# DIAGNijmegen/spgnn

Measured on NVIDIA B200. Metric: spgnn3_train_graphs_per_s, higher is better.
Workload: dtype f32

## Files before the change

### include/spgnn_b200.h

```cpp
#ifndef SPGNN_B200_H
#define SPGNN_B200_H

#include <stdint.h>

#ifdef __cplusplus
extern "C" {
#endif

#define SPGNN_OK            0
#define SPGNN_E_INVALID    -1
#define SPGNN_E_CUDA       -2
#define SPGNN_E_UNSUPPORTED -3
#define SPGNN_E_WORKSPACE  -4

#define SPGNN_ACT_NONE 0
#define SPGNN_ACT_ELU  1
#define SPGNN_ACT_TANH 2
#define SPGNN_ACT_RELU 3
#define SPGNN_ACT_LEAKY 4

const char* spgnn_last_error(void);
int  spgnn_abi_version(void);
int64_t spgnn_launch_count(void);
int  spgnn_device_info(int* sm_count, int* cc_major, int* cc_minor);
// ... 36 lines not shown
                       float p, uint64_t seed, int64_t concat_chunks, int64_t chunk_off,
                       uint16_t* out_hi, int64_t ldo, int64_t plane_stride, int64_t M, void* stream);
int64_t spgnn_planes_linear_fwd_ws(int64_t N, int64_t K1, int64_t K2);
int spgnn_planes_linear_fwd(const uint16_t* A1, int64_t lda1, int64_t ps1, int64_t K1,
                            const uint16_t* A2, int64_t lda2, int64_t ps2, int64_t K2,
                            const float* W, int64_t ldw, const float* bias, int act, float slope,
                            float* C, int64_t ldc, int64_t M, int64_t N, void* ws, int64_t ws_bytes, void* stream);
int64_t spgnn_planes_linear_bwd_input_ws(int64_t N, int64_t K);
int spgnn_planes_linear_bwd_input(const uint16_t* dC, int64_t lddc, int64_t ps, const float* W, int64_t ldw,
                                  int64_t k_off, float* dA, int64_t ldda, int64_t M, int64_t N, int64_t K,
                                  void* ws, int64_t ws_bytes, void* stream);
int spgnn_planes_linear_bwd_input_masked(const uint16_t* dC, int64_t lddc, int64_t ps, const float* W, int64_t ldw,
                                         int64_t k_off, float* dA, int64_t ldda, int64_t M, int64_t N, int64_t K,
                                         float drop_p, uint64_t seed, int64_t concat_chunks,
                                         void* ws, int64_t ws_bytes, void* stream);
int64_t spgnn_planes_linear_bwd_weight_ws(int64_t M, int64_t N, int64_t K1, int64_t K2);
int spgnn_planes_linear_bwd_weight(const uint16_t* dC, int64_t lddc, int64_t psc,
                                   const uint16_t* X1, int64_t ldx1, int64_t psx1, int64_t K1,
                                   const uint16_t* X2, int64_t ldx2, int64_t psx2, int64_t K2,
                                   float* dW, int64_t lddw, int64_t M, int64_t N,
                                   void* ws, int64_t ws_bytes, void* stream);
int64_t spgnn_act_bwd_planes_ws(int64_t N);
int spgnn_act_bwd_planes(const float* g, int64_t ldg, const float* y, int64_t ldy, int act, float slope,
                         float drop_p, uint64_t drop_seed, uint16_t* out_hi, int64_t ldo, int64_t plane_stride,
                         int64_t M, int64_t N, float* colsum_out, void* ws, void* stream);
int64_t spgnn_planes_linear_bwd_weight_plan(int64_t M, int64_t N, int64_t K1, int64_t K2, int32_t* out, int64_t cap);

int64_t spgnn_colsum_ws(int64_t N);
int spgnn_colsum(const float* X, int64_t ldx, int64_t M, int64_t N, float* out, void* ws, void* stream);

// ... 68 lines not shown
    float* d_eler; int64_t ld_de;
    uint16_t* d_eler_planes; int64_t ld_dep; int64_t ps_dep;
    float* dX; int64_t ld_dx;
} spgnn_gat_wide;
int64_t spgnn_gat_wide_sizeof(void);
int spgnn_gat_aggx_fwd(const spgnn_gat_wide* L, void* stream);
int spgnn_gat_aggx_bwd(const spgnn_gat_wide* L, void* stream);

int64_t spgnn_wide_linear_ws(int64_t H, int64_t F, int64_t kp, int has_res);
int spgnn_wide_linear(const uint16_t* XA, int64_t ldxa, int64_t psxa, int64_t kp, int64_t k_in, int64_t M,
                      int H, int F, int has_res, const float* W, int64_t ldw, const float* bias, int act, int mode,
                      float* out, int64_t ldo, uint16_t* out_planes, int64_t ldp, int64_t psp,
                      const float* g0, int64_t ldg0, const float* g1, int64_t ldg1, const float* g2, int64_t ldg2,
                      uint16_t* dpre, int64_t ldd, int64_t psd, float* dbias,
                      void* ws, int64_t ws_bytes, void* stream);

int spgnn_spmm(const float* x, int64_t ldx, const int32_t* ptr, const int32_t* nbr,
               const float* pre, const float* post, const float* self_eps_ptr,
               const float* bias, int act, float slope,
               float* out, int64_t ldo, int64_t N, int64_t F, void* stream);
int spgnn_degree_norms(const int32_t* ptr, int64_t N, float* norm_sqrt, float* norm_inv, void* stream);

int spgnn_sage_maxpool_fwd(const float* m, int64_t ldm, const int32_t* in_ptr, const int32_t* in_src,
                           float* out, int64_t ldo, int32_t* arg, int64_t N, int64_t F, void* stream);
int spgnn_sage_maxpool_bwd(const float* g, int64_t ldg, const int32_t* arg,
                           const int32_t* out_ptr, const int32_t* out_dst, const int32_t* out_slot,
                           float* dm, int64_t lddm, int64_t N, int64_t F, void* stream);

int spgnn_bias_act(const float* x, int64_t ldx, const float* bias, int act, float slope,
                   float* y, int64_t ldy, int64_t M, int64_t N, void* stream);
// ... 58 lines not shown
```

### spgnn_b200/csrc/gemm_tma.cu

```cuda
#include "common.cuh"
#include "tc_ptx.cuh"

namespace spgnn {
namespace tma {
using namespace ptx;

constexpr int BM = 128;
constexpr int BK = 64;
constexpr int kThreads = 192;
constexpr int kEpiWarps = 4;
constexpr int kMaxStages = 6;
constexpr int kMaxBN = 256;
constexpr int kABytes = BM * 128 * 2;
constexpr int kStgLd = 36;
constexpr int kStgBytes = kEpiWarps * 32 * kStgLd * 4;
constexpr int kSmemLimit = 232448;
constexpr int kNtFixed = 1024  + 256  + kStgBytes;

__device__ __forceinline__ float4 ld_shared4(uint32_t addr) {
    float4 v;
    asm volatile("ld.shared.v4.f32 {%0, %1, %2, %3}, [%4];" : "=f"(v.x), "=f"(v.y), "=f"(v.z), "=f"(v.w) : "r"(addr));
    return v;
}
__device__ __forceinline__ void st_shared4(uint32_t addr, uint32_t a, uint32_t b, uint32_t c, uint32_t d) {
    asm volatile("st.shared.v4.b32 [%0], {%1, %2, %3, %4};" ::"r"(addr), "r"(a), "r"(b), "r"(c), "r"(d) : "memory");
}

struct NtMaps { CUtensorMap a1, a2, b; };
struct NtArgs {
    const float* bias; int act; float slope;
    float* C; int64_t ldc;
    int64_t M; int N;
    int BN, nt_n; int64_t nt_m;
    int kb1, kb2;
    int stages, stage_bytes;
    uint32_t mthr; float mscale; uint64_t mseed; int64_t mnch, moff;
};
__device__ __forceinline__ float4 nt_mask4(const NtArgs& g, float4 x, int64_t row, int col) {
    const uint64_t h = chunk_hash(g.mseed, (uint64_t)row * (uint64_t)g.mnch + (uint64_t)(g.moff + (col >> 2)));
    x.x = ((uint32_t)(h) & 0xFFFFu) >= g.mthr ? x.x * g.mscale : 0.f;
    x.y = ((uint32_t)(h >> 16) & 0xFFFFu) >= g.mthr ? x.y * g.mscale : 0.f;
    x.z = ((uint32_t)(h >> 32) & 0xFFFFu) >= g.mthr ? x.z * g.mscale : 0.f;
    x.w = ((uint32_t)(h >> 48) & 0xFFFFu) >= g.mthr ? x.w * g.mscale : 0.f;
    return x;
}
struct NtShared {
    uint64_t full[kMaxStages];
    uint64_t empty[kMaxStages];
    uint64_t tmem_full[2];
    uint64_t tmem_empty[2];
    uint32_t tmem_base;
// ... 47 lines not shown
                if (g.mthr) x = nt_mask4(g, x, row0 + 4 * itr, col);
                float* qq = q + itr * qstep;
                if (vec_ok && nvalid >= 4) st4(qq, x);
                else {
                    if (nvalid > 0) qq[0] = x.x;
                    if (nvalid > 1) qq[1] = x.y;
                    if (nvalid > 2) qq[2] = x.z;
                    if (nvalid > 3) qq[3] = x.w;
                }
            }
        }
        __syncwarp();
    }
}

template <int CL>
__global__ void __launch_bounds__(kThreads, 1) nt_planes_kernel(const __grid_constant__ NtMaps maps, const NtArgs g) {
    extern __shared__ uint8_t smem_raw[];
    uint8_t* smem = reinterpret_cast<uint8_t*>(((uintptr_t)smem_raw + 1023) & ~(uintptr_t)1023);
    const int stages_bytes = g.stages * g.stage_bytes;
    NtShared* sh = reinterpret_cast<NtShared*>(smem + stages_bytes);
    const int warp = threadIdx.x >> 5, lane = threadIdx.x & 31;
    const uint32_t smem_base = smem_u32(smem);

    if (threadIdx.x == 0) {
        for (int s = 0; s < g.stages; ++s) {
            mbar_init(smem_u32(&sh->full[s]), 1);
            mbar_init(smem_u32(&sh->empty[s]), CL);
        }
        for (int b = 0; b < 2; ++b) {
// ... 12 lines not shown
    __syncthreads();
    if (CL > 1) cluster_sync_all();
    tc_fence_after();
    const uint32_t tmem_base = sh->tmem_base;

    const int rank = CL > 1 ? (int)cluster_ctarank() : 0;
    const int64_t n_tiles = (CL > 1 ? (g.nt_m + CL - 1) / CL : g.nt_m) * g.nt_n;
    const int64_t tile0 = blockIdx.x / CL, tile_step = gridDim.x / CL;
    const int nkb = g.kb1 + g.kb2;

    if (warp < kEpiWarps) {
        int it = 0;
        const uint32_t stg = smem_base + stages_bytes + 256 + warp * (32 * kStgLd * 4);
        const bool vec_ok = (g.ldc % 4 == 0) && ((reinterpret_cast<uintptr_t>(g.C) & 15) == 0);
        const bool plain = (g.act == SPGNN_ACT_NONE) && (g.bias == nullptr);
        for (int64_t tile = tile0; tile < n_tiles; tile += tile_step, ++it) {
            const int buf = it & 1;
            const uint32_t par = (it >> 1) & 1;
            const int64_t m0 = ((tile / g.nt_n) * CL + rank) * BM;
            const int n0 = (int)(tile % g.nt_n) * g.BN;
            const int ncols = min(g.BN, g.N - n0);
            mbar_wait(smem_u32(&sh->tmem_full[buf]), par);
            tc_fence_after();
            const uint32_t taddr = tmem_base + ((uint32_t)(warp * 32) << 16) + (uint32_t)(buf * kMaxBN);
            nt_epilogue_tile(g, stg, taddr, m0, n0, ncols, warp, lane, vec_ok, plain);
            tc_fence_before();
            mbar_arrive(smem_u32(&sh->tmem_empty[buf]));
        }
    } else if (warp == kEpiWarps) {
        {
            int it = 0;
            uint32_t kcount = 0;
            const uint32_t tbase = __shfl_sync(kFull, tmem_base, 0);
            for (int64_t tile = tile0; tile < n_tiles; tile += tile_step, ++it) {
                const int buf = it & 1;
                const uint32_t par = (it >> 1) & 1;
                const int n0 = (int)(tile % g.nt_n) * g.BN;
                const int ncols = min(g.BN, g.N - n0);
                const int n_mma = (ncols + 15) & ~15;
                const uint32_t idesc = make_idesc(n_mma, false);
// ... 187 lines not shown
    if (warp == kEpiWarps) {
        tc_fence_after();
        tmem_dealloc_pair(tmem_base, 512);
    }
}

struct WideMaps { CUtensorMap a, b; };
struct WideArgs {
    int mode, H, F, act;
    const float* bias;
    float* out; int64_t ldo;
    __nv_bfloat16* outp; int64_t ldp, psp;
    const float* g[3]; int64_t ldg[3]; int n_g;
    __nv_bfloat16* dpre; int64_t ldd, psd;
    float* dbias_ws;
    int64_t M; int BN, nt_n; int64_t nt_m;
    int kbp, nparts, kp;
    int stages, stage_bytes;
};
constexpr int kWideEpiWarps = 16;
constexpr int kWideThreads = (kWideEpiWarps + 2) * 32;
constexpr int kWideStgBytes = kWideEpiWarps * 32 * 16 * 4;
constexpr int kWideFixed = 1024  + 256  + kWideStgBytes;

template <int ACT>
__device__ __forceinline__ float wide_act(float x, int act) {
    if (ACT == SPGNN_ACT_ELU) return x > 0.f ? x : exp_fast(x) - 1.f;
    if (ACT == SPGNN_ACT_NONE) return x;
    return act_fwd(x, act, 0.f);
}
template <int ACT>
__device__ __forceinline__ float wide_act_grad(float y, int act) {
    if (ACT == SPGNN_ACT_ELU) return y > 0.f ? 1.f : y + 1.f;
    if (ACT == SPGNN_ACT_NONE) return 1.f;
    return act_grad_from_out(y, act, 0.f);
}
template <int ACT>
__device__ __forceinline__ float wide_act_grad_pre(float x, int act) {
    if (ACT == SPGNN_ACT_ELU) return x > 0.f ? 1.f : exp_fast(x);
    if (ACT == SPGNN_ACT_NONE) return 1.f;
    return act_grad_from_out(act_fwd(x, act, 0.f), act, 0.f);
}
__device__ __forceinline__ void st_planes4(__nv_bfloat16* q, int64_t ps, float4 d) {
    uint32_t h0, l0, h1, l1;
    split2(d.x, d.y, h0, l0);
    split2(d.z, d.w, h1, l1);
    *reinterpret_cast<uint2*>(q) = make_uint2(h0, h1);
    *reinterpret_cast<uint2*>(q + ps) = make_uint2(l0, l1);
}
template <int ACT, int MODE>
__device__ __forceinline__ void wide_epilogue_tile(const WideArgs& g, uint32_t stg, float* dbias_row, uint32_t taddr,
                                                   int64_t m0, int n0, int ncols, int warp, int lane,
                                                   uint32_t full_bar, uint32_t full_par) {
    const int quad = warp & 3, part = warp >> 2;
    const int r0 = lane >> 2, cq = lane & 3;
    const float inv_h = 1.f / (float)g.H;
    const int64_t row0 = m0 + quad * 32 + r0;
    const int nrow = (int)max((int64_t)0, min((int64_t)4, (g.M - row0 + 7) / 8));
    const uint32_t st_w = stg + lane * 64;
    const int sw_w = (lane >> 1) & 3;
    uint32_t st_r[4];
#pragma unroll
    for (int i = 0; i < 4; ++i) {
// ... 35 lines not shown
                for (int i = 0; i < 4; ++i) {
                    run[q][i].x *= inv_h; run[q][i].y *= inv_h; run[q][i].z *= inv_h; run[q][i].w *= inv_h;
                }
        }
        if (cg == 0) {
            mbar_wait(full_bar, full_par);
            tc_fence_after();
        }
#pragma unroll
        for (int q = 0; q < 2; ++q) {
            const int c0 = cg + q * 64 + part * 16;
            if (c0 >= ncols) break;
            const int col = colq + c0;
            __nv_bfloat16* dp = MODE == 1 ? g.dpre + row0 * g.ldd + col : nullptr;
            const int64_t dstep = 8 * g.ldd;
            uint32_t v[16];
            tmem_ld16(taddr + c0, v);
            for (int h = 0; h < g.H; ++h) {
                const float4 bv = g.bias ? ldg4(g.bias + h * g.F + col) : make_float4(0.f, 0.f, 0.f, 0.f);
                tmem_ld_wait();
#pragma unroll
                for (int j = 0; j < 4; ++j)
                    st_shared4(st_w + ((j ^ sw_w) << 4), v[4 * j], v[4 * j + 1], v[4 * j + 2], v[4 * j + 3]);
                __syncwarp();
                if (h + 1 < g.H) tmem_ld16(taddr + (h + 1) * g.BN + c0, v);
                float4 bs = make_float4(0.f, 0.f, 0.f, 0.f);
#pragma unroll
                for (int i = 0; i < 4; ++i) {
                    float4 x = ld_shared4(st_r[i]);
                    if (MODE == 0) {
                        run[q][i].x += wide_act<ACT>(x.x + bv.x, g.act);
                        run[q][i].y += wide_act<ACT>(x.y + bv.y, g.act);
                        run[q][i].z += wide_act<ACT>(x.z + bv.z, g.act);
                        run[q][i].w += wide_act<ACT>(x.w + bv.w, g.act);
                    } else if (i < nrow) {
                        float4 d;
                        d.x = run[q][i].x * wide_act_grad_pre<ACT>(x.x + bv.x, g.act);
                        d.y = run[q][i].y * wide_act_grad_pre<ACT>(x.y + bv.y, g.act);
                        d.z = run[q][i].z * wide_act_grad_pre<ACT>(x.z + bv.z, g.act);
                        d.w = run[q][i].w * wide_act_grad_pre<ACT>(x.w + bv.w, g.act);
                        st_planes4(dp + i * dstep + h * g.F, g.psd, d);
                        bs.x += d.x; bs.y += d.y; bs.z += d.z; bs.w += d.w;
                    }
                }
                if (MODE == 1 && dbias_row) {
#pragma unroll
                    for (int o = 4; o < 32; o <<= 1) {
                        bs.x += __shfl_xor_sync(kFull, bs.x, o); bs.y += __shfl_xor_sync(kFull, bs.y, o);
                        bs.z += __shfl_xor_sync(kFull, bs.z, o); bs.w += __shfl_xor_sync(kFull, bs.w, o);
// ... 782 lines not shown
    const int64_t ldb = k1p + k2p;
    __nv_bfloat16* hi = reinterpret_cast<__nv_bfloat16*>(((uintptr_t)ws + 127) & ~(uintptr_t)127);
    split_weight_kernel<<<split_grid(N * ldb), 256, 0, st>>>(W, ldw, 0, 0, (int)N, (int)ldb, (int)K1, k1p, (int)K2, 0,
                                                             hi, hi + N * ldb, ldb);
    SPGNN_LAUNCH_OK();
    return launch_nt(reinterpret_cast<const __nv_bfloat16*>(A1), lda1, ps1, K1,
                     reinterpret_cast<const __nv_bfloat16*>(A2), lda2, ps2, K2, hi, ldb, bias, act, slope, C, ldc, M, N,
                     st);
}

extern "C" int64_t spgnn_wide_linear_ws(int64_t H, int64_t F, int64_t kp, int has_res) {
    const int64_t b = 2 * H * F * (has_res ? 2 : 1) * kp * (int64_t)sizeof(__nv_bfloat16);
    return b + 256 + (int64_t)sm_count() * H * F * (int64_t)sizeof(float) + 256;
}

extern "C" int spgnn_wide_linear(const uint16_t* XA, int64_t ldxa, int64_t psxa, int64_t kp, int64_t k_in, int64_t M,
                                 int H, int F, int has_res, const float* W, int64_t ldw, const float* bias, int act,
                                 int mode, float* out, int64_t ldo, uint16_t* out_planes, int64_t ldp, int64_t psp,
                                 const float* g0, int64_t ldg0, const float* g1, int64_t ldg1, const float* g2,
                                 int64_t ldg2, uint16_t* dpre, int64_t ldd, int64_t psd, float* dbias, void* ws,
                                 int64_t ws_bytes, void* stream) {
    SPGNN_REQUIRE(XA && W && ws && M > 0 && k_in > 0, "wide_linear: bad argument");
    SPGNN_REQUIRE(H == 1 || H == 2 || H == 4, "wide_linear: H must be 1, 2 or 4 (got %d)", H);
    SPGNN_REQUIRE(F > 0 && F % 32 == 0 && (int64_t)H * F <= 8192, "wide_linear: F (%d) must be a multiple of 32, H*F <= 8192", F);
    SPGNN_REQUIRE(kp % BK == 0 && kp >= k_in && ldxa >= (H + 1) * kp && ldw >= k_in, "wide_linear: kp / ld mismatch");
    SPGNN_REQUIRE(mode == 0 || mode == 1, "wide_linear: mode must be 0 (forward) or 1 (gradient of the pre-activations)");
    SPGNN_REQUIRE(!bias || ((uintptr_t)bias & 15) == 0, "wide_linear: bias must be 16-byte aligned");
    SPGNN_REQUIRE(ws_bytes >= spgnn_wide_linear_ws(H, F, kp, has_res), "wide_linear: workspace too small");
    SPGNN_REQUIRE(M < (1ll << 31), "wide_linear: too many rows");
    WideMaps maps;
    WideArgs a{};
    a.mode = mode; a.H = H; a.F = F; a.act = act; a.bias = bias; a.M = M;
    if (mode == 0) {
        SPGNN_REQUIRE(out || out_planes, "wide_linear: no output");
        SPGNN_REQUIRE(!out || (ldo % 4 == 0 && ldo >= F && ((uintptr_t)out & 15) == 0), "wide_linear: out alignment");
        SPGNN_REQUIRE(!out_planes || (ldp % 4 == 0 && ldp >= F && psp % 4 == 0 && ((uintptr_t)out_planes & 7) == 0),
                      "wide_linear: out planes alignment");
        a.out = out; a.ldo = ldo; a.outp = reinterpret_cast<__nv_bfloat16*>(out_planes); a.ldp = ldp; a.psp = psp;
    } else {
        SPGNN_REQUIRE(g0 && dpre, "wide_linear: mode 1 needs a gradient source and the dpre planes");
        SPGNN_REQUIRE(ldd % 4 == 0 && ldd >= (int64_t)H * F && psd % 4 == 0 && ((uintptr_t)dpre & 7) == 0,
                      "wide_linear: dpre planes alignment");
        const float* gs[3] = {g0, g1, g2};
        const int64_t lds[3] = {ldg0, ldg1, ldg2};
        for (int s = 0; s < 3; ++s) {
            if (!gs[s]) continue;
            SPGNN_REQUIRE(lds[s] % 4 == 0 && lds[s] >= F && ((uintptr_t)gs[s] & 15) == 0,
                          "wide_linear: gradient source %d must be 16-byte aligned with ld %% 4 == 0", s);
            a.g[a.n_g] = gs[s]; a.ldg[a.n_g] = lds[s]; ++a.n_g;
        }
        a.dpre = reinterpret_cast<__nv_bfloat16*>(dpre); a.ldd = ldd; a.psd = psd;
    }
    cudaStream_t st = as_stream(stream);
    static DeviceOnce attr;
// ... 46 lines not shown
        at[0].id = cudaLaunchAttributeClusterDimension;
        at[0].val.clusterDim.x = 2; at[0].val.clusterDim.y = 1; at[0].val.clusterDim.z = 1;
        cfg.gridDim = dim3(grid); cfg.blockDim = dim3(kWideThreads);
        cfg.dynamicSmemBytes = kSmemLimit; cfg.stream = st; cfg.attrs = at; cfg.numAttrs = 1;
        SPGNN_CUDA_OK(cudaLaunchKernelEx(&cfg, wide_pair_kernel, maps, a));
        count_launch();
    } else {
        wide_kernel<<<grid, kWideThreads, kSmemLimit, st>>>(maps, a);
        SPGNN_LAUNCH_OK();
    }
    if (part) {
        wide_dbias_reduce_kernel<<<(unsigned)ceil_div(HF, 128), 128, 0, st>>>(part, grid, HF, dbias);
        SPGNN_LAUNCH_OK();
    }
    return SPGNN_OK;
}

extern "C" int64_t spgnn_planes_linear_bwd_input_ws(int64_t N, int64_t K) {
    return 2 * K * (int64_t)round_up(N, BK) * 2 + 256;
}

extern "C" int spgnn_planes_linear_bwd_input(const uint16_t* dC, int64_t lddc, int64_t ps, const float* W, int64_t ldw,
                                             int64_t k_off, float* dA, int64_t ldda, int64_t M, int64_t N, int64_t K,
                                             void* ws, int64_t ws_bytes, void* stream) {
    return spgnn_planes_linear_bwd_input_masked(dC, lddc, ps, W, ldw, k_off, dA, ldda, M, N, K, 0.f, 0, 0, ws, ws_bytes,
                                                stream);
}

extern "C" int spgnn_planes_linear_bwd_input_masked(const uint16_t* dC, int64_t lddc, int64_t ps, const float* W,
                                                    int64_t ldw, int64_t k_off, float* dA, int64_t ldda, int64_t M,
                                                    int64_t N, int64_t K, float drop_p, uint64_t seed,
                                                    int64_t concat_chunks, void* ws, int64_t ws_bytes, void* stream) {
    SPGNN_REQUIRE(dC && W && dA && ws && M > 0 && N > 0 && K > 0, "planes_linear_bwd_input: bad argument");
    SPGNN_REQUIRE(drop_p >= 0.f && drop_p < 1.f, "planes_linear_bwd_input: dropout p");
    SPGNN_REQUIRE(drop_p == 0.f || k_off % 4 == 0, "planes_linear_bwd_input: a masked output needs k_off %% 4 == 0");
    SPGNN_REQUIRE(ldw >= k_off + K && ldda >= K, "planes_linear_bwd_input: leading dimension too small");
    SPGNN_REQUIRE(ws_bytes >= spgnn_planes_linear_bwd_input_ws(N, K), "planes_linear_bwd_input: workspace too small");
    cudaStream_t st = as_stream(stream);
    const int np = round_up(N, BK);
    __nv_bfloat16* hi = reinterpret_cast<__nv_bfloat16*>(((uintptr_t)ws + 127) & ~(uintptr_t)127);
    split_weight_kernel<<<split_grid(K * np), 256, 0, st>>>(W, ldw, 1, k_off, (int)K, np, 0, 0, 0, (int)N, hi,
                                                            hi + K * np, np);
    SPGNN_LAUNCH_OK();
    return launch_nt(reinterpret_cast<const __nv_bfloat16*>(dC), lddc, ps, N, nullptr, 0, 0, 0, hi, np, nullptr, 0, 0.f,
                     dA, ldda, M, K, st, drop_p, seed, concat_chunks > 0 ? concat_chunks : (k_off + K + 3) / 4, k_off / 4);
}

namespace {
struct TnPlan {
    bool swap;
    int npb, nqb, np_tiles, nq_tiles;
    int64_t splits, rows;
    double cost;
};
int blocks_of(int64_t c0, int64_t c1, int* valid) {
    int n = 0;
    for (int64_t c : {c0, c1})
        for (int64_t o = 0; o < c; o += 64) valid[n++] = (int)(c - o < 64 ? c - o : 64);
    return n;
}
// ... 182 lines not shown
```

### spgnn_b200/stack.py

```python
from __future__ import annotations

import ctypes
import os

import torch
from torch.autograd import Function

from . import ops
from ._lib import SpgnnError, lib, ptr, stream


class _Sink(ctypes.Structure):
    _fields_ = [("hi", ctypes.c_void_p), ("ld", ctypes.c_int64), ("plane_stride", ctypes.c_int64),
                ("concat_chunks", ctypes.c_int64), ("chunk_off", ctypes.c_int64),
                ("drop_p", ctypes.c_float), ("reserved", ctypes.c_uint32), ("seed", ctypes.c_uint64)]


class _GSrc(ctypes.Structure):
    _fields_ = [("g", ctypes.c_void_p), ("ld", ctypes.c_int64), ("concat_chunks", ctypes.c_int64),
                ("chunk_off", ctypes.c_int64), ("drop_p", ctypes.c_float), ("reserved", ctypes.c_uint32),
                ("seed", ctypes.c_uint64)]


class _Layer(ctypes.Structure):
# ... 27 lines not shown
                ("eler", ctypes.c_void_p), ("ld_eler", ctypes.c_int64),
                ("negative_slope", ctypes.c_float), ("attn_drop_p", ctypes.c_float), ("attn_seed", ctypes.c_uint64),
                ("att", ctypes.c_void_p),
                ("XA", ctypes.c_void_p), ("ldxa", ctypes.c_int64), ("psxa", ctypes.c_int64), ("kp", ctypes.c_int64),
                ("dXA", ctypes.c_void_p), ("ld_dxa", ctypes.c_int64), ("head_stride", ctypes.c_int64),
                ("w_eler", ctypes.c_void_p), ("ld_w", ctypes.c_int64),
                ("ds_ws", ctypes.c_void_p),
                ("d_eler", ctypes.c_void_p), ("ld_de", ctypes.c_int64),
                ("d_eler_planes", ctypes.c_void_p), ("ld_dep", ctypes.c_int64), ("ps_dep", ctypes.c_int64),
                ("dX", ctypes.c_void_p), ("ld_dx", ctypes.c_int64)]


WIDE_OUTPUT_LAYER = True
TREE_KERNELS = True
FOLD_MASK = os.environ.get("SPGNN_FOLD_MASK", "1") != "0"

_checked = False


def _check_abi():
    global _checked
    if not _checked:
        n = int(lib().gat_layer_sizeof())
        if n != ctypes.sizeof(_Layer):
            raise SpgnnError(f"spgnn_gat_layer layout mismatch: library {n} bytes, binding {ctypes.sizeof(_Layer)}")
        n = int(lib().gat_wide_sizeof())
        if n != ctypes.sizeof(_Wide):
            raise SpgnnError(f"spgnn_gat_wide layout mismatch: library {n} bytes, binding {ctypes.sizeof(_Wide)}")
        _checked = True

# ... 177 lines not shown
                    raise SpgnnError(f"stack: tensor {t!r} consumed before it is produced")
                variants[key] = split_planes(ext[t], pdrop[i], fseed[i], nch, off // 4)
            ins.append(variants[key])
        cons = plan.consumers.get(L.output, [])
        keys = []
        for ci, _ in cons:
            if vkey[ci] not in keys:
                keys.append(vkey[ci])
        is_out = L.output in plan.outputs
        want_head = head is not None and L.output == plan.outputs[0]
        if want_head and -1 not in keys:
            keys.append(-1)
        if len(keys) > 2:
            raise SpgnnError("stack: more than two dropout variants of one tensor are not supported")
        if L.wide and WIDE_OUTPUT_LAYER and all(k < 0 for k in keys):
            out32, P, rec = _wide_forward(L, graph, ins, packed[i], biases[i], conv, training, aseed[i], is_out,
                                          bool(keys))
            if P is not None:
                variants[(L.output, -1)] = P
            if is_out:
                outs[L.output] = out32
            if want_head:
                emb_planes = P
            if keep:
                tape.layers[i] = rec
            for t in L.inputs:
                if all(ci <= i for ci, _ in plan.consumers[t]):
                    for k in [k for k in variants if k[0] == t]:
                        del variants[k]
            continue
        Y = planes_linear(ins[0], packed[i], A2=ins[1] if len(ins) > 1 else None)
        d = _Layer()
# ... 38 lines not shown
        if keep:
            tape.layers[i] = (ins, Y, att, b)
        for t in L.inputs:
            if all(ci <= i for ci, _ in plan.consumers[t]):
                for k in [k for k in variants if k[0] == t]:
                    del variants[k]
    logits = None
    if head is not None:
        logits = planes_linear(emb_planes, head[0], head[1])
        if keep:
            tape.emb_planes = emb_planes
    return logits, outs, tape


class _WideRec:
    __slots__ = ("XA", "att", "eler", "bias", "aseed", "kp")


def _wide_desc(L, graph, conv, training, aseed, XA, kp, eler, att):
    d = _Wide()
    d.in_ptr, d.in_src = ptr(graph.in_ptr), ptr(graph.in_src)
    d.out_ptr, d.out_dst, d.out_slot = ptr(graph.out_ptr), ptr(graph.out_dst), ptr(graph.out_slot)
    d.N, d.H, d.has_res = graph.num_nodes, L.H, int(L.res_mode == 1)
    d.eler, d.ld_eler = ptr(eler), eler.stride(0)
    d.negative_slope = conv.negative_slope
    d.attn_drop_p = conv.attn_drop_p if training else 0.0
    d.attn_seed = aseed
    d.att = ptr(att)
    d.XA, d.ldxa, d.psxa, d.kp = XA.ptr(), XA.ld, XA.ps, kp
    return d


def _wide_forward(L, graph, ins, W, bias, conv, training, aseed, want_out, want_planes):
    L_ = lib()
    dev = graph.in_ptr.device
    N, E, H, F = graph.num_nodes, graph.num_edges, L.H, L.F
    hf, k_in = H * F, L.k_in
    has_res = int(L.res_mode == 1)
    kp = (k_in + 63) // 64 * 64
    rows0 = hf * (1 + has_res)
    eler = planes_linear(ins[0], W[rows0:rows0 + 2 * H], A2=ins[1] if len(ins) > 1 else None)
    XA = Planes(N, (H + 1) * kp, dev)
    att = torch.empty(E, H, dtype=torch.float32, device=dev)
    d = _wide_desc(L, graph, conv, training, aseed, XA, kp, eler, att)
    if ops.tracing():
        ops.trace_gat(graph, eler[:, :H], eler[:, H:2 * H], d.attn_drop_p, aseed)
    d.X1, d.ldx1, d.psx1, d.K1 = ins[0].ptr(), ins[0].ld, ins[0].ps, ins[0].cols
    if len(ins) > 1:
        d.X2, d.ldx2, d.psx2, d.K2 = ins[1].ptr(), ins[1].ld, ins[1].ps, ins[1].cols
    L_.gat_aggx_fwd(ctypes.byref(d), stream(),
                    _key=("bytes", 4.0 * N * (k_in + 2 * H) + 4.0 * N * (H + 1) * kp + 4.0 * (N + 1) + 4.0 * E))
    out32 = ops.empty_padded(N, F, dev) if want_out else None
    P = Planes(N, F, dev) if want_planes else None
    ws = _ws(L_.wide_linear_ws(H, F, kp, has_res), dev)
    L_.wide_linear(XA.ptr(), XA.ld, XA.ps, kp, k_in, N, H, F, has_res, ptr(W), W.stride(0), ptr(bias), conv._act, 0,
                   ptr(out32), out32.stride(0) if out32 is not None else 0,
                   P.ptr() if P is not None else None, P.ld if P is not None else 0, P.ps if P is not None else 0,
                   None, 0, None, 0, None, 0, None, 0, 0, None, ptr(ws), ws.numel(), stream(),
                   _key=("flops", 2.0 * N * hf * k_in * (1 + has_res)))
    rec = _WideRec()
    rec.XA, rec.att, rec.eler, rec.bias, rec.aseed, rec.kp = XA, att, eler, bias, aseed, kp
    return out32, P, rec


def _wide_backward(L, graph, rec, W, gsrcs, training, need_bias):
    L_ = lib()
    dev = graph.in_ptr.device
    N, E, H, F = graph.num_nodes, graph.num_edges, L.H, L.F
    hf, k_in, kp = H * F, L.k_in, rec.kp
    k4 = (k_in + 3) // 4 * 4
    has_res = int(L.res_mode == 1)
    conv = L.conv
    if not 1 <= len(gsrcs) <= 3:
        raise SpgnnError("stack: 1..3 gradient contributions to the output layer are supported")
    XA = rec.XA
    dpre = Planes(N, hf, dev)
    db = torch.empty(hf, dtype=torch.float32, device=dev) if rec.bias is not None and need_bias else None
    ws = _ws(L_.wide_linear_ws(H, F, kp, has_res), dev)
    gp = [(ptr(g), g.stride(0)) for g in gsrcs] + [(None, 0)] * (3 - len(gsrcs))
    L_.wide_linear(XA.ptr(), XA.ld, XA.ps, kp, k_in, N, H, F, has_res, ptr(W), W.stride(0), ptr(rec.bias), conv._act, 1,
                   None, 0, None, 0, 0, gp[0][0], gp[0][1], gp[1][0], gp[1][1], gp[2][0], gp[2][1],
                   dpre.ptr(), dpre.ld, dpre.ps, ptr(db), ptr(ws), ws.numel(), stream(),
                   _key=("flops", 2.0 * N * hf * k_in * (1 + has_res)))
    ldx = (1 + has_res) * k4
    dXA = torch.empty(H, N, ldx, dtype=torch.float32, device=dev)
    x_view = PlanesView(XA, H * kp, k_in)
    dWz, dWres = [], []
    pad = k4 - k_in
    for h in range(H):
        dpre_h = PlanesView(dpre, h * F, F)
        dW_h = planes_linear_bwd_weight(dpre_h, PlanesView(XA, h * kp, k_in), x_view if has_res else None)
        dWz.append(dW_h[:, :k_in])
        blocks = [W[h * F:(h + 1) * F]] + ([W[hf + h * F:hf + (h + 1) * F]] if has_res else [])
        if pad:
            blocks = [torch.nn.functional.pad(b_, (0, pad)) for b_ in blocks]
        Wcat = torch.cat(blocks, 1) if len(blocks) > 1 else blocks[0].contiguous()
        planes_linear_bwd_input(dpre_h, Wcat, ldx, out=dXA[h])
        if has_res:
# ... 42 lines not shown
    L_ = lib()
    dev = graph.in_ptr.device
    N, E = graph.num_nodes, graph.num_edges
    nL = len(plan.layers)
    d_packed, d_bias = [None] * nL, [None] * nL
    d_hw = d_hb = None
    extra = {}
    for name, g in g_outs.items():
        if g is not None:
            extra.setdefault(name, []).append(_grad_rows(g))
    if head is not None and g_logits is not None:
        gl = _grad_rows(g_logits)
        glp = split_planes(gl)
        d_hw = planes_linear_bwd_weight(glp, tape.emb_planes)
        d_hb = ops.colsum(gl)
        extra.setdefault(plan.outputs[0], []).append(planes_linear_bwd_input(glp, head[0], head[0].shape[1]))
        tape.emb_planes = None
    dX = {}
    masked = set()
    for i in range(nL - 1, -1, -1):
        L = plan.layers[i]
        conv = L.conv
        srcs = []
        for ci, off in plan.consumers.get(L.output, []):
            if ci in dX and dX[ci] is not None and off < dX[ci].shape[1]:
                pm = 0.0 if ci in masked else tape.pdrop[ci]
                srcs.append((dX[ci], off, pm, tape.fseed[ci], (plan.layers[ci].k_in + 3) // 4))
        for g in extra.get(L.output, []):
            srcs.append((g, 0, 0.0, 0, 1))
        if not srcs:
            dX[i] = None
            tape.layers[i] = None
            continue
        if len(srcs) > 3:
            raise SpgnnError("stack: more than three gradient contributions to one tensor are not supported")
        hf = L.H * L.F
        if isinstance(tape.layers[i], _WideRec):
            rec = tape.layers[i]
            tape.layers[i] = None
            if any(p > 0.0 or off for _, off, p, _, _ in srcs):
                raise SpgnnError("stack: a head-averaged output layer cannot have masked gradient sources")
            d_packed[i], d_bias[i], dX[i] = _wide_backward(L, graph, rec, packed[i], [g for g, *_ in srcs],
                                                           tape.training, need_bias[i])
            continue
        ins, Y, att, b = tape.layers[i]
# ... 103 lines not shown
```

Measured before the change: 51660.

## Fuse head backward-input GEMM with wide layer dpre computation via saved activation grads

During training, the wide output layer's forward epilogue now also stores the per-head activation derivative (dact) in fp32. The head's backward-input GEMM then has a custom epilogue that multiplies the gradient by dact/H per head. It writes the dpre bf16 planes and per-block dbias partials directly. This skips the separate wide_linear mode-1 backward pass, which recomputed the forward GEMM to get activation derivatives. In exchange it adds an N×H×F fp32 dact write and read, plus atomics for the bias partials.

```diff
diff --git a/include/spgnn_b200.h b/include/spgnn_b200.h
--- a/include/spgnn_b200.h
+++ b/include/spgnn_b200.h
@@ -74,6 +74,11 @@
                                          int64_t k_off, float* dA, int64_t ldda, int64_t M, int64_t N, int64_t K,
                                          float drop_p, uint64_t seed, int64_t concat_chunks,
                                          void* ws, int64_t ws_bytes, void* stream);
+int64_t spgnn_planes_linear_bwd_input_dpre_ws(int64_t N, int64_t H, int64_t F);
+int spgnn_planes_linear_bwd_input_dpre(const uint16_t* dC, int64_t lddc, int64_t ps, const float* W, int64_t ldw,
+                                       int64_t M, int64_t N, int H, int F, const float* dact, int64_t ld_dact,
+                                       uint16_t* dpre, int64_t ldd, int64_t psd, float* dbias,
+                                       void* ws, int64_t ws_bytes, void* stream);
 int64_t spgnn_planes_linear_bwd_weight_ws(int64_t M, int64_t N, int64_t K1, int64_t K2);
 int spgnn_planes_linear_bwd_weight(const uint16_t* dC, int64_t lddc, int64_t psc,
                                    const uint16_t* X1, int64_t ldx1, int64_t psx1, int64_t K1,
@@ -172,6 +177,10 @@
                       const float* g0, int64_t ldg0, const float* g1, int64_t ldg1, const float* g2, int64_t ldg2,
                       uint16_t* dpre, int64_t ldd, int64_t psd, float* dbias,
                       void* ws, int64_t ws_bytes, void* stream);
+int spgnn_wide_linear_fwd_dact(const uint16_t* XA, int64_t ldxa, int64_t psxa, int64_t kp, int64_t k_in, int64_t M,
+                               int H, int F, int has_res, const float* W, int64_t ldw, const float* bias, int act,
+                               float* out, int64_t ldo, uint16_t* out_planes, int64_t ldp, int64_t psp,
+                               float* dact, int64_t ld_dact, void* ws, int64_t ws_bytes, void* stream);
 
 int spgnn_spmm(const float* x, int64_t ldx, const int32_t* ptr, const int32_t* nbr,
                const float* pre, const float* post, const float* self_eps_ptr,
diff --git a/spgnn_b200/csrc/gemm_tma.cu b/spgnn_b200/csrc/gemm_tma.cu
--- a/spgnn_b200/csrc/gemm_tma.cu
+++ b/spgnn_b200/csrc/gemm_tma.cu
@@ -25,6 +25,13 @@
 __device__ __forceinline__ void st_shared4(uint32_t addr, uint32_t a, uint32_t b, uint32_t c, uint32_t d) {
     asm volatile("st.shared.v4.b32 [%0], {%1, %2, %3, %4};" ::"r"(addr), "r"(a), "r"(b), "r"(c), "r"(d) : "memory");
 }
+__device__ __forceinline__ void st_planes4(__nv_bfloat16* q, int64_t ps, float4 d) {
+    uint32_t h0, l0, h1, l1;
+    split2(d.x, d.y, h0, l0);
+    split2(d.z, d.w, h1, l1);
+    *reinterpret_cast<uint2*>(q) = make_uint2(h0, h1);
+    *reinterpret_cast<uint2*>(q + ps) = make_uint2(l0, l1);
+}
 
 struct NtMaps { CUtensorMap a1, a2, b; };
 struct NtArgs {
@@ -35,6 +42,9 @@
     int kb1, kb2;
     int stages, stage_bytes;
     uint32_t mthr; float mscale; uint64_t mseed; int64_t mnch, moff;
+    const float* dact; int64_t ldact;
+    __nv_bfloat16* dpre; int64_t ldd, psd;
+    float* dbias_ws; int dH;
 };
 __device__ __forceinline__ float4 nt_mask4(const NtArgs& g, float4 x, int64_t row, int col) {
     const uint64_t h = chunk_hash(g.mseed, (uint64_t)row * (uint64_t)g.mnch + (uint64_t)(g.moff + (col >> 2)));
@@ -112,6 +122,81 @@
     }
 }
 
+template <int NH>
+__device__ __forceinline__ void nt_dpre_tile(const NtArgs& g, uint32_t stg, float* dbias_row, uint32_t taddr,
+                                             int64_t m0, int n0, int ncols, int warp, int lane, uint32_t full_bar,
+                                             uint32_t full_par) {
+    constexpr int RB = NH == 4 ? 4 : 8;
+    const float inv_h = 1.f / (float)NH;
+    const int cc = (lane & 7) * 4;
+    const int rsub = lane >> 3;
+    const int64_t row0 = m0 + warp * 32 + rsub;
+    const int nrow = (int)max((int64_t)0, min((int64_t)8, (g.M - row0 + 3) / 4));
+    const uint32_t sp = stg + (rsub * kStgLd + cc) * 4;
+    for (int c0 = 0; c0 < ncols; c0 += 32) {
+        const bool cok = c0 + cc < ncols;
+        const int col = n0 + c0 + cc;
+        const float* pa = g.dact + row0 * g.ldact + col;
+        __nv_bfloat16* pd = g.dpre + row0 * g.ldd + col;
+        float4 bs[NH];
+#pragma unroll
+        for (int h = 0; h < NH; ++h) bs[h] = make_float4(0.f, 0.f, 0.f, 0.f);
+#pragma unroll
+        for (int rb = 0; rb < 8; rb += RB) {
+            float4 a[NH][RB];
+#pragma unroll
+            for (int h = 0; h < NH; ++h)
+#pragma unroll
+                for (int r = 0; r < RB; ++r)
+                    if (rb + r < nrow && cok) a[h][r] = ldg4(pa + (rb + r) * 4 * g.ldact + h * g.N);
+            if (rb == 0) {
+                if (c0 == 0) {
+                    mbar_wait(full_bar, full_par);
+                    tc_fence_after();
+                }
+                uint32_t v[32];
+                tmem_ld16(taddr + c0, *reinterpret_cast<uint32_t(*)[16]>(&v[0]));
+                tmem_ld16(taddr + c0 + 16, *reinterpret_cast<uint32_t(*)[16]>(&v[16]));
+                tmem_ld_wait();
+#pragma unroll
+                for (int j = 0; j < 8; ++j)
+                    st_shared4(stg + (lane * kStgLd + 4 * j) * 4, v[4 * j], v[4 * j + 1], v[4 * j + 2], v[4 * j + 3]);
+                __syncwarp();
+            }
+#pragma unroll
+            for (int r = 0; r < RB; ++r) {
+                const int itr = rb + r;
+                if (itr < nrow && cok) {
+                    float4 x = ld_shared4(sp + itr * (4 * kStgLd * 4));
+                    x.x *= inv_h; x.y *= inv_h; x.z *= inv_h; x.w *= inv_h;
+#pragma unroll
+                    for (int h = 0; h < NH; ++h) {
+                        float4 d;
+                        d.x = x.x * a[h][r].x; d.y = x.y * a[h][r].y; d.z = x.z * a[h][r].z; d.w = x.w * a[h][r].w;
+                        st_planes4(pd + itr * 4 * g.ldd + h * g.N, g.psd, d);
+                        bs[h].x += d.x; bs[h].y += d.y; bs[h].z += d.z; bs[h].w += d.w;
+                    }
+                }
+            }
+        }
+        if (dbias_row) {
+#pragma unroll
+            for (int h = 0; h < NH; ++h) {
+#pragma unroll
+                for (int o = 8; o < 32; o <<= 1) {
+                    bs[h].x += __shfl_xor_sync(kFull, bs[h].x, o); bs[h].y += __shfl_xor_sync(kFull, bs[h].y, o);
+                    bs[h].z += __shfl_xor_sync(kFull, bs[h].z, o); bs[h].w += __shfl_xor_sync(kFull, bs[h].w, o);
+                }
+                if (lane < 8 && cok) {
+                    float* p = dbias_row + h * g.N + col;
+                    atomicAdd(p, bs[h].x); atomicAdd(p + 1, bs[h].y); atomicAdd(p + 2, bs[h].z); atomicAdd(p + 3, bs[h].w);
+                }
+            }
+        }
+        __syncwarp();
+    }
+}
+
 template <int CL>
 __global__ void __launch_bounds__(kThreads, 1) nt_planes_kernel(const __grid_constant__ NtMaps maps, const NtArgs g) {
     extern __shared__ uint8_t smem_raw[];
@@ -154,16 +239,24 @@
         const uint32_t stg = smem_base + stages_bytes + 256 + warp * (32 * kStgLd * 4);
         const bool vec_ok = (g.ldc % 4 == 0) && ((reinterpret_cast<uintptr_t>(g.C) & 15) == 0);
         const bool plain = (g.act == SPGNN_ACT_NONE) && (g.bias == nullptr);
+        float* dbias_row = g.dbias_ws ? g.dbias_ws + (int64_t)blockIdx.x * (g.dH * g.N) : nullptr;
         for (int64_t tile = tile0; tile < n_tiles; tile += tile_step, ++it) {
             const int buf = it & 1;
             const uint32_t par = (it >> 1) & 1;
             const int64_t m0 = ((tile / g.nt_n) * CL + rank) * BM;
             const int n0 = (int)(tile % g.nt_n) * g.BN;
             const int ncols = min(g.BN, g.N - n0);
-            mbar_wait(smem_u32(&sh->tmem_full[buf]), par);
-            tc_fence_after();
             const uint32_t taddr = tmem_base + ((uint32_t)(warp * 32) << 16) + (uint32_t)(buf * kMaxBN);
-            nt_epilogue_tile(g, stg, taddr, m0, n0, ncols, warp, lane, vec_ok, plain);
+            if (CL == 1 && g.dpre) {
+                const uint32_t fb = smem_u32(&sh->tmem_full[buf]);
+                if (g.dH == 1) nt_dpre_tile<1>(g, stg, dbias_row, taddr, m0, n0, ncols, warp, lane, fb, par);
+                else if (g.dH == 2) nt_dpre_tile<2>(g, stg, dbias_row, taddr, m0, n0, ncols, warp, lane, fb, par);
+                else nt_dpre_tile<4>(g, stg, dbias_row, taddr, m0, n0, ncols, warp, lane, fb, par);
+            } else {
+                mbar_wait(smem_u32(&sh->tmem_full[buf]), par);
+                tc_fence_after();
+                nt_epilogue_tile(g, stg, taddr, m0, n0, ncols, warp, lane, vec_ok, plain);
+            }
             tc_fence_before();
             mbar_arrive(smem_u32(&sh->tmem_empty[buf]));
         }
@@ -381,6 +474,7 @@
     const float* g[3]; int64_t ldg[3]; int n_g;
     __nv_bfloat16* dpre; int64_t ldd, psd;
     float* dbias_ws;
+    float* dact; int64_t ldact;
     int64_t M; int BN, nt_n; int64_t nt_m;
     int kbp, nparts, kp;
     int stages, stage_bytes;
@@ -407,13 +501,6 @@
     if (ACT == SPGNN_ACT_ELU) return x > 0.f ? 1.f : exp_fast(x);
     if (ACT == SPGNN_ACT_NONE) return 1.f;
     return act_grad_from_out(act_fwd(x, act, 0.f), act, 0.f);
-}
-__device__ __forceinline__ void st_planes4(__nv_bfloat16* q, int64_t ps, float4 d) {
-    uint32_t h0, l0, h1, l1;
-    split2(d.x, d.y, h0, l0);
-    split2(d.z, d.w, h1, l1);
-    *reinterpret_cast<uint2*>(q) = make_uint2(h0, h1);
-    *reinterpret_cast<uint2*>(q + ps) = make_uint2(l0, l1);
 }
 template <int ACT, int MODE>
 __device__ __forceinline__ void wide_epilogue_tile(const WideArgs& g, uint32_t stg, float* dbias_row, uint32_t taddr,
@@ -479,6 +566,8 @@
             const int col = colq + c0;
             __nv_bfloat16* dp = MODE == 1 ? g.dpre + row0 * g.ldd + col : nullptr;
             const int64_t dstep = 8 * g.ldd;
+            float* sp = MODE == 0 && g.dact ? g.dact + m0 * g.ldact : nullptr;
+            const uint32_t so = (uint32_t)((row0 - m0) * g.ldact + col), sstep = (uint32_t)(8 * g.ldact);
             uint32_t v[16];
             tmem_ld16(taddr + c0, v);
             for (int h = 0; h < g.H; ++h) {
@@ -498,6 +587,12 @@
                         run[q][i].y += wide_act<ACT>(x.y + bv.y, g.act);
                         run[q][i].z += wide_act<ACT>(x.z + bv.z, g.act);
                         run[q][i].w += wide_act<ACT>(x.w + bv.w, g.act);
+                        if (sp && i < nrow)
+                            st4(sp + (so + i * sstep + h * g.F),
+                                make_float4(wide_act_grad_pre<ACT>(x.x + bv.x, g.act),
+                                            wide_act_grad_pre<ACT>(x.y + bv.y, g.act),
+                                            wide_act_grad_pre<ACT>(x.z + bv.z, g.act),
+                                            wide_act_grad_pre<ACT>(x.w + bv.w, g.act)));
                     } else if (i < nrow) {
                         float4 d;
                         d.x = run[q][i].x * wide_act_grad_pre<ACT>(x.x + bv.x, g.act);
@@ -1310,12 +1405,12 @@
     return b + 256 + (int64_t)sm_count() * H * F * (int64_t)sizeof(float) + 256;
 }
 
-extern "C" int spgnn_wide_linear(const uint16_t* XA, int64_t ldxa, int64_t psxa, int64_t kp, int64_t k_in, int64_t M,
-                                 int H, int F, int has_res, const float* W, int64_t ldw, const float* bias, int act,
-                                 int mode, float* out, int64_t ldo, uint16_t* out_planes, int64_t ldp, int64_t psp,
-                                 const float* g0, int64_t ldg0, const float* g1, int64_t ldg1, const float* g2,
-                                 int64_t ldg2, uint16_t* dpre, int64_t ldd, int64_t psd, float* dbias, void* ws,
-                                 int64_t ws_bytes, void* stream) {
+static int wide_linear(const uint16_t* XA, int64_t ldxa, int64_t psxa, int64_t kp, int64_t k_in, int64_t M, int H,
+                       int F, int has_res, const float* W, int64_t ldw, const float* bias, int act, int mode, float* out,
+                       int64_t ldo, uint16_t* out_planes, int64_t ldp, int64_t psp, float* dact, int64_t ld_dact,
+                       const float* g0, int64_t ldg0, const float* g1, int64_t ldg1, const float* g2, int64_t ldg2,
+                       uint16_t* dpre, int64_t ldd, int64_t psd, float* dbias, void* ws, int64_t ws_bytes,
+                       void* stream) {
     SPGNN_REQUIRE(XA && W && ws && M > 0 && k_in > 0, "wide_linear: bad argument");
     SPGNN_REQUIRE(H == 1 || H == 2 || H == 4, "wide_linear: H must be 1, 2 or 4 (got %d)", H);
     SPGNN_REQUIRE(F > 0 && F % 32 == 0 && (int64_t)H * F <= 8192, "wide_linear: F (%d) must be a multiple of 32, H*F <= 8192", F);
@@ -1333,7 +1428,11 @@
         SPGNN_REQUIRE(!out_planes || (ldp % 4 == 0 && ldp >= F && psp % 4 == 0 && ((uintptr_t)out_planes & 7) == 0),
                       "wide_linear: out planes alignment");
         a.out = out; a.ldo = ldo; a.outp = reinterpret_cast<__nv_bfloat16*>(out_planes); a.ldp = ldp; a.psp = psp;
+        SPGNN_REQUIRE(!dact || (ld_dact % 4 == 0 && ld_dact >= (int64_t)H * F && ((uintptr_t)dact & 15) == 0),
+                      "wide_linear: dact must be 16-byte aligned with ld %% 4 == 0 and ld >= H*F");
+        a.dact = dact; a.ldact = ld_dact;
     } else {
+        SPGNN_REQUIRE(!dact, "wide_linear: dact is an output of mode 0");
         SPGNN_REQUIRE(g0 && dpre, "wide_linear: mode 1 needs a gradient source and the dpre planes");
         SPGNN_REQUIRE(ldd % 4 == 0 && ldd >= (int64_t)H * F && psd % 4 == 0 && ((uintptr_t)dpre & 7) == 0,
                       "wide_linear: dpre planes alignment");
@@ -1410,6 +1509,26 @@
         SPGNN_LAUNCH_OK();
     }
     return SPGNN_OK;
+}
+
+extern "C" int spgnn_wide_linear(const uint16_t* XA, int64_t ldxa, int64_t psxa, int64_t kp, int64_t k_in, int64_t M,
+                                 int H, int F, int has_res, const float* W, int64_t ldw, const float* bias, int act,
+                                 int mode, float* out, int64_t ldo, uint16_t* out_planes, int64_t ldp, int64_t psp,
+                                 const float* g0, int64_t ldg0, const float* g1, int64_t ldg1, const float* g2,
+                                 int64_t ldg2, uint16_t* dpre, int64_t ldd, int64_t psd, float* dbias, void* ws,
+                                 int64_t ws_bytes, void* stream) {
+    return wide_linear(XA, ldxa, psxa, kp, k_in, M, H, F, has_res, W, ldw, bias, act, mode, out, ldo, out_planes, ldp,
+                       psp, nullptr, 0, g0, ldg0, g1, ldg1, g2, ldg2, dpre, ldd, psd, dbias, ws, ws_bytes, stream);
+}
+
+extern "C" int spgnn_wide_linear_fwd_dact(const uint16_t* XA, int64_t ldxa, int64_t psxa, int64_t kp, int64_t k_in,
+                                          int64_t M, int H, int F, int has_res, const float* W, int64_t ldw,
+                                          const float* bias, int act, float* out, int64_t ldo, uint16_t* out_planes,
+                                          int64_t ldp, int64_t psp, float* dact, int64_t ld_dact, void* ws,
+                                          int64_t ws_bytes, void* stream) {
+    SPGNN_REQUIRE(dact, "wide_linear_fwd_dact: no dact");
+    return wide_linear(XA, ldxa, psxa, kp, k_in, M, H, F, has_res, W, ldw, bias, act, 0, out, ldo, out_planes, ldp, psp,
+                       dact, ld_dact, nullptr, 0, nullptr, 0, nullptr, 0, nullptr, 0, 0, nullptr, ws, ws_bytes, stream);
 }
 
 extern "C" int64_t spgnn_planes_linear_bwd_input_ws(int64_t N, int64_t K) {
@@ -1440,6 +1559,71 @@
     SPGNN_LAUNCH_OK();
     return launch_nt(reinterpret_cast<const __nv_bfloat16*>(dC), lddc, ps, N, nullptr, 0, 0, 0, hi, np, nullptr, 0, 0.f,
                      dA, ldda, M, K, st, drop_p, seed, concat_chunks > 0 ? concat_chunks : (k_off + K + 3) / 4, k_off / 4);
+}
+
+extern "C" int64_t spgnn_planes_linear_bwd_input_dpre_ws(int64_t N, int64_t H, int64_t F) {
+    return spgnn_planes_linear_bwd_input_ws(N, F) + (int64_t)sm_count() * H * F * (int64_t)sizeof(float) + 256;
+}
+
+extern "C" int spgnn_planes_linear_bwd_input_dpre(const uint16_t* dC, int64_t lddc, int64_t ps, const float* W,
+                                                  int64_t ldw, int64_t M, int64_t N, int H, int F, const float* dact,
+                                                  int64_t ld_dact, uint16_t* dpre, int64_t ldd, int64_t psd,
+                                                  float* dbias, void* ws, int64_t ws_bytes, void* stream) {
+    SPGNN_REQUIRE(dC && W && dact && dpre && ws && M > 0 && N > 0, "planes_linear_bwd_input_dpre: bad argument");
+    SPGNN_REQUIRE(N <= BK, "planes_linear_bwd_input_dpre: N (%lld) must be <= %d", (long long)N, BK);
+    SPGNN_REQUIRE(H == 1 || H == 2 || H == 4, "planes_linear_bwd_input_dpre: H must be 1, 2 or 4 (got %d)", H);
+    SPGNN_REQUIRE(F > 0 && F % 32 == 0, "planes_linear_bwd_input_dpre: F (%d) must be a multiple of 32", F);
+    SPGNN_REQUIRE(ldw >= F && M < (1ll << 31), "planes_linear_bwd_input_dpre: shape");
+    SPGNN_REQUIRE(ld_dact % 4 == 0 && ld_dact >= (int64_t)H * F && ((uintptr_t)dact & 15) == 0,
+                  "planes_linear_bwd_input_dpre: dact must be 16-byte aligned with ld %% 4 == 0 and ld >= H*F");
+    SPGNN_REQUIRE(ldd % 4 == 0 && ldd >= (int64_t)H * F && psd % 4 == 0 && ((uintptr_t)dpre & 7) == 0,
+                  "planes_linear_bwd_input_dpre: dpre planes alignment");
+    SPGNN_REQUIRE(ws_bytes >= spgnn_planes_linear_bwd_input_dpre_ws(N, H, F),
+                  "planes_linear_bwd_input_dpre: workspace too small");
+    cudaStream_t st = as_stream(stream);
+    static DeviceOnce attr;
+    if (attr.pending()) {
+        SPGNN_CUDA_OK(cudaFuncSetAttribute(nt_planes_kernel<1>, cudaFuncAttributeMaxDynamicSharedMemorySize, kSmemLimit));
+        attr.done();
+    }
+    const int np = round_up(N, BK);
+    __nv_bfloat16* hi = reinterpret_cast<__nv_bfloat16*>(((uintptr_t)ws + 127) & ~(uintptr_t)127);
+    split_weight_kernel<<<split_grid((int64_t)F * np), 256, 0, st>>>(W, ldw, 1, 0, F, np, 0, 0, 0, (int)N, hi,
+                                                                     hi + (int64_t)F * np, np);
+    SPGNN_LAUNCH_OK();
+    NtMaps maps;
+    NtArgs a{};
+    pick_bn(F, &a.BN, &a.nt_n);
+    int rc = make_planes_map(&maps.a1, dC, M, N, lddc, ps, BK, BM);
+    if (rc) return rc;
+    maps.a2 = maps.a1;
+    rc = make_planes_map(&maps.b, hi, F, np, np, (int64_t)F * np, BK, a.BN);
+    if (rc) return rc;
+    a.act = SPGNN_ACT_NONE; a.M = M; a.N = F;
+    a.mscale = 1.f; a.mnch = (F + 3) / 4;
+    a.nt_m = ceil_div(M, BM);
+    a.kb1 = 1;
+    a.stage_bytes = kABytes + a.BN * 256;
+    a.stages = (kSmemLimit - kNtFixed) / a.stage_bytes;
+    if (a.stages > kMaxStages) a.stages = kMaxStages;
+    a.dact = dact; a.ldact = ld_dact;
+    a.dpre = reinterpret_cast<__nv_bfloat16*>(dpre); a.ldd = ldd; a.psd = psd; a.dH = H;
+    const int64_t tiles = a.nt_m * a.nt_n;
+    const unsigned grid = (unsigned)(tiles < sm_count() ? tiles : sm_count());
+    const int64_t HF = (int64_t)H * F;
+    float* part = nullptr;
+    if (dbias) {
+        part = reinterpret_cast<float*>(((uintptr_t)(hi + 2 * (int64_t)F * np) + 255) & ~(uintptr_t)255);
+        a.dbias_ws = part;
+        SPGNN_CUDA_OK(cudaMemsetAsync(part, 0, (size_t)grid * HF * sizeof(float), st));
+    }
+    nt_planes_kernel<1><<<grid, kThreads, kSmemLimit, st>>>(maps, a);
+    SPGNN_LAUNCH_OK();
+    if (part) {
+        wide_dbias_reduce_kernel<<<(unsigned)ceil_div(HF, 128), 128, 0, st>>>(part, grid, HF, dbias);
+        SPGNN_LAUNCH_OK();
+    }
+    return SPGNN_OK;
 }
 
 namespace {
diff --git a/spgnn_b200/stack.py b/spgnn_b200/stack.py
--- a/spgnn_b200/stack.py
+++ b/spgnn_b200/stack.py
@@ -65,6 +65,7 @@
 WIDE_OUTPUT_LAYER = True
 TREE_KERNELS = True
 FOLD_MASK = os.environ.get("SPGNN_FOLD_MASK", "1") != "0"
+DPRE_EPILOGUE = os.environ.get("SPGNN_DPRE_EPILOGUE", "1") != "0"
 
 _checked = False
 
@@ -272,8 +273,9 @@
         if len(keys) > 2:
             raise SpgnnError("stack: more than two dropout variants of one tensor are not supported")
         if L.wide and WIDE_OUTPUT_LAYER and all(k < 0 for k in keys):
+            slopes = keep and training and DPRE_EPILOGUE and want_head and not cons
             out32, P, rec = _wide_forward(L, graph, ins, packed[i], biases[i], conv, training, aseed[i], is_out,
-                                          bool(keys))
+                                          bool(keys), slopes)
             if P is not None:
                 variants[(L.output, -1)] = P
             if is_out:
@@ -342,7 +344,7 @@
 
 
 class _WideRec:
-    __slots__ = ("XA", "att", "eler", "bias", "aseed", "kp")
+    __slots__ = ("XA", "att", "eler", "bias", "aseed", "kp", "dact", "dpre", "db")
 
 
 def _wide_desc(L, graph, conv, training, aseed, XA, kp, eler, att):
@@ -359,7 +361,7 @@
     return d
 
 
-def _wide_forward(L, graph, ins, W, bias, conv, training, aseed, want_out, want_planes):
+def _wide_forward(L, graph, ins, W, bias, conv, training, aseed, want_out, want_planes, want_dact=False):
     L_ = lib()
     dev = graph.in_ptr.device
     N, E, H, F = graph.num_nodes, graph.num_edges, L.H, L.F
@@ -381,14 +383,36 @@
     out32 = ops.empty_padded(N, F, dev) if want_out else None
     P = Planes(N, F, dev) if want_planes else None
     ws = _ws(L_.wide_linear_ws(H, F, kp, has_res), dev)
-    L_.wide_linear(XA.ptr(), XA.ld, XA.ps, kp, k_in, N, H, F, has_res, ptr(W), W.stride(0), ptr(bias), conv._act, 0,
-                   ptr(out32), out32.stride(0) if out32 is not None else 0,
-                   P.ptr() if P is not None else None, P.ld if P is not None else 0, P.ps if P is not None else 0,
-                   None, 0, None, 0, None, 0, None, 0, 0, None, ptr(ws), ws.numel(), stream(),
-                   _key=("flops", 2.0 * N * hf * k_in * (1 + has_res)))
+    outs = (ptr(out32), out32.stride(0) if out32 is not None else 0,
+            P.ptr() if P is not None else None, P.ld if P is not None else 0, P.ps if P is not None else 0)
+    dact = None
+    if want_dact:
+        dact = torch.empty(N, hf, dtype=torch.float32, device=dev)
+        L_.wide_linear_fwd_dact(XA.ptr(), XA.ld, XA.ps, kp, k_in, N, H, F, has_res, ptr(W), W.stride(0), ptr(bias),
+                                conv._act, *outs, ptr(dact), dact.stride(0), ptr(ws), ws.numel(), stream(),
+                                _key=("flops", 2.0 * N * hf * k_in * (1 + has_res)), _name="wide_linear")
+    else:
+        L_.wide_linear(XA.ptr(), XA.ld, XA.ps, kp, k_in, N, H, F, has_res, ptr(W), W.stride(0), ptr(bias), conv._act, 0,
+                       *outs, None, 0, None, 0, None, 0, None, 0, 0, None, ptr(ws), ws.numel(), stream(),
+                       _key=("flops", 2.0 * N * hf * k_in * (1 + has_res)))
     rec = _WideRec()
     rec.XA, rec.att, rec.eler, rec.bias, rec.aseed, rec.kp = XA, att, eler, bias, aseed, kp
+    rec.dact, rec.dpre, rec.db = dact, None, None
     return out32, P, rec
+
+
+def _head_dpre(L, rec, glp, head_w, need_bias):
+    L_ = lib()
+    N, H, F = glp.rows, L.H, L.F
+    W = ops._rows(head_w)
+    dpre = Planes(N, H * F, W.device)
+    db = torch.empty(H * F, dtype=torch.float32, device=W.device) if rec.bias is not None and need_bias else None
+    ws = _ws(L_.planes_linear_bwd_input_dpre_ws(glp.cols, H, F), W.device)
+    L_.planes_linear_bwd_input_dpre(glp.ptr(), glp.ld, glp.ps, ptr(W), W.stride(0), N, glp.cols, H, F, ptr(rec.dact),
+                                    rec.dact.stride(0), dpre.ptr(), dpre.ld, dpre.ps, ptr(db), ptr(ws), ws.numel(),
+                                    stream(), _key=("bytes", 4.0 * N * glp.cols + 8.0 * N * H * F + 4.0 * N * H * F))
+    rec.dact = None
+    rec.dpre, rec.db = dpre, db
 
 
 def _wide_backward(L, graph, rec, W, gsrcs, training, need_bias):
@@ -399,17 +423,24 @@
     k4 = (k_in + 3) // 4 * 4
     has_res = int(L.res_mode == 1)
     conv = L.conv
-    if not 1 <= len(gsrcs) <= 3:
-        raise SpgnnError("stack: 1..3 gradient contributions to the output layer are supported")
     XA = rec.XA
-    dpre = Planes(N, hf, dev)
-    db = torch.empty(hf, dtype=torch.float32, device=dev) if rec.bias is not None and need_bias else None
-    ws = _ws(L_.wide_linear_ws(H, F, kp, has_res), dev)
-    gp = [(ptr(g), g.stride(0)) for g in gsrcs] + [(None, 0)] * (3 - len(gsrcs))
-    L_.wide_linear(XA.ptr(), XA.ld, XA.ps, kp, k_in, N, H, F, has_res, ptr(W), W.stride(0), ptr(rec.bias), conv._act, 1,
-                   None, 0, None, 0, 0, gp[0][0], gp[0][1], gp[1][0], gp[1][1], gp[2][0], gp[2][1],
-                   dpre.ptr(), dpre.ld, dpre.ps, ptr(db), ptr(ws), ws.numel(), stream(),
-                   _key=("flops", 2.0 * N * hf * k_in * (1 + has_res)))
+    if rec.dpre is not None:
+        if gsrcs:
+            raise SpgnnError("stack: the output layer's dpre came from the head, yet it has further gradients")
+        dpre, db = rec.dpre, rec.db
+        rec.dpre = rec.db = None
+    else:
+        if not 1 <= len(gsrcs) <= 3:
+            raise SpgnnError("stack: 1..3 gradient contributions to the output layer are supported")
+        rec.dact = None
+        dpre = Planes(N, hf, dev)
+        db = torch.empty(hf, dtype=torch.float32, device=dev) if rec.bias is not None and need_bias else None
+        ws = _ws(L_.wide_linear_ws(H, F, kp, has_res), dev)
+        gp = [(ptr(g), g.stride(0)) for g in gsrcs] + [(None, 0)] * (3 - len(gsrcs))
+        L_.wide_linear(XA.ptr(), XA.ld, XA.ps, kp, k_in, N, H, F, has_res, ptr(W), W.stride(0), ptr(rec.bias),
+                       conv._act, 1, None, 0, None, 0, 0, gp[0][0], gp[0][1], gp[1][0], gp[1][1], gp[2][0], gp[2][1],
+                       dpre.ptr(), dpre.ld, dpre.ps, ptr(db), ptr(ws), ws.numel(), stream(),
+                       _key=("flops", 2.0 * N * hf * k_in * (1 + has_res)))
     ldx = (1 + has_res) * k4
     dXA = torch.empty(H, N, ldx, dtype=torch.float32, device=dev)
     x_view = PlanesView(XA, H * kp, k_in)
@@ -482,7 +513,14 @@
         glp = split_planes(gl)
         d_hw = planes_linear_bwd_weight(glp, tape.emb_planes)
         d_hb = ops.colsum(gl)
-        extra.setdefault(plan.outputs[0], []).append(planes_linear_bwd_input(glp, head[0], head[0].shape[1]))
+        name = plan.outputs[0]
+        io = plan.producer.get(name)
+        rec = tape.layers[io] if io is not None else None
+        if (isinstance(rec, _WideRec) and rec.dact is not None and name not in extra
+                and not plan.consumers.get(name)):
+            _head_dpre(plan.layers[io], rec, glp, head[0], need_bias[io])
+        else:
+            extra.setdefault(name, []).append(planes_linear_bwd_input(glp, head[0], head[0].shape[1]))
         tape.emb_planes = None
     dX = {}
     masked = set()
@@ -496,7 +534,7 @@
                 srcs.append((dX[ci], off, pm, tape.fseed[ci], (plan.layers[ci].k_in + 3) // 4))
         for g in extra.get(L.output, []):
             srcs.append((g, 0, 0.0, 0, 1))
-        if not srcs:
+        if not srcs and not (isinstance(tape.layers[i], _WideRec) and tape.layers[i].dpre is not None):
             dX[i] = None
             tape.layers[i] = None
             continue
```

New measurement: 52860 (median of 6 runs). +2.3%, better.
